# tusen-ai/SST

Hardware: AMD Instinct MI355X
Metric: LiDAR frames/sec (SST backbone fwd+bwd) at Waymo 0.32m voxels (higher is better)
Workload: dtype f32 (storage, accumulation, attention, LayerNorm, reductions: fp32; the dense products of the encoder layers from the EXACT three-way bf16 split of both fp32 operands, six bf16 MFMA products with fp32 accumulation - error vs float64 <= 2 x the fp32 matrix pipe's: tests/test_gpu_dense_f32x6.py)

## Files before the change

sst_amd/csrc/layer_exec.hip:

```cpp
#include <stdint.h>
#include "common.h"

namespace {

enum { kEpiBias = 0, kEpiGelu = 1, kEpiRelu = 2, kEpiMulGeluGrad = 3, kEpiMulReluGrad = 4, kEpiAdd = 5 };
constexpr int kC = 128, kFF = 256;

int64_t wg_ws(int64_t m, int which) {
  sst_wgrad_problem_f32 p[5];
  float* const any = (float*)(uintptr_t)256;
  for (auto& q : p) {
    q.dy = q.x = any;
    q.dw = q.db = any;
    q.m = m;
    q.x_add_rows = nullptr, q.x_add_index = nullptr;
  }
  if (which == 0 || which == 2) {
    p[0].ld_dy = kC, p[0].ld_x = kFF, p[0].out = kC, p[0].in = kFF;
    p[1].ld_dy = kFF, p[1].ld_x = kC, p[1].out = kFF, p[1].in = kC;
    if (which == 0) return sst_weight_grad_group_f32x6_workspace_bytes(p, 2);
    p[2].ld_dy = kC, p[2].ld_x = kC, p[2].out = kC, p[2].in = kC;
    p[3].ld_dy = 3 * kC, p[3].ld_x = kC, p[3].out = 2 * kC, p[3].in = kC;
    p[4].ld_dy = 3 * kC, p[4].ld_x = kC, p[4].out = kC, p[4].in = kC;
    return sst_weight_grad_group_f32x6_workspace_bytes(p, 5);
// ... 1 lines not shown
  p[0].ld_dy = kC, p[0].ld_x = kC, p[0].out = kC, p[0].in = kC;
  p[1].ld_dy = 3 * kC, p[1].ld_x = kC, p[1].out = 2 * kC, p[1].in = kC;
  p[2].ld_dy = 3 * kC, p[2].ld_x = kC, p[2].out = kC, p[2].in = kC;
  return sst_weight_grad_group_f32x6_workspace_bytes(p, 3);
}

int64_t wg_ws_bf16(int64_t m) {
  sst_wgrad_problem_bf16 p[5];
  for (auto& q : p) q.m = m;
  p[0].p = 2 * kC, p[1].p = kC, p[2].p = kC, p[3].p = kFF, p[4].p = kFF;
  return sst_wgrad_group_workspace_bytes(p, 5);
}

}

extern "C" {

int64_t sst_encoder_layer_bwd_workspace_bytes(int64_t m, int n_heads) {
  if (m < 0 || n_heads < 1) return SST_ERR_ARG;
  const int64_t a = sst_encoder_tail_bwd_workspace_bytes(m), d = sst_sra_attn_bwd_workspace_bytes(m, n_heads), e = wg_ws(m, 2);
  if (a < 0 || d < 0 || e < 0) return SST_ERR_UNSUPPORTED;
  return sst_align_up(a, 256) + sst_align_up(e, 256) + sst_align_up(d, 256) + 256;
}

int64_t sst_encoder_layer_wpack_bytes(void) { return sst_encoder_tail_pack_bytes(); }

int sst_encoder_layer_fwd_f32x6(const sst_encoder_layer_fwd_args* a, void* stream) {
  if (!a || a->m < 0 || a->n_heads * 16 != kC || (a->act != 1 && a->act != 2)) return SST_ERR_ARG;
  if (a->m == 0) return SST_OK;
  if (!a->x || !a->qkv || !a->o || !a->lse || !a->y1 || !a->st1 || !a->pre || !a->h || !a->s2 || !a->y2 || !a->st2)
    return SST_ERR_ARG;
  if (!a->xp && (!a->xpos_table || !a->xpos_idx)) return SST_ERR_ARG;
  const int64_t m = a->m;
  int rc;
  if (a->xp == nullptr)
    rc = sst_inproj_pos_f32x6(a->x, kC, a->xpos_table, a->xpos_idx, a->w_in, kC, a->b_in, m, a->qkv, 3 * kC, stream);
  else
    rc = sst_tall_linear_epi2_f32x6(a->xp, a->x, 2 * kC, kC, a->w_in, kC, 0, a->b_in, m, kC, 3 * kC, kEpiBias, nullptr, nullptr, 0,
                                    a->qkv, 3 * kC, stream);
  if (rc) return rc;
  if (a->head_scale != nullptr)
    rc = sst_sra_attn_cos_fwd_f32(a->qkv, a->qkv + kC, a->qkv + 2 * kC, 3 * kC, 3 * kC, 3 * kC, a->tok, a->winoff, a->order,
                                  a->n_windows, a->n_heads, a->head_scale, a->max_tokens, a->o, kC, a->lse, stream);
  else
    rc = sst_sra_attn_fwd_ord_f32(a->qkv, a->qkv + kC, a->qkv + 2 * kC, 3 * kC, 3 * kC, 3 * kC, a->tok, a->winoff, a->order,
                                  a->n_windows, a->n_heads, a->scale, a->max_tokens, a->impl, a->o, kC, a->lse, stream);
  if (rc) return rc;
  if (!a->wpack) return SST_ERR_ARG;
  if (a->w_out || a->w1 || a->w2) {
    rc = sst_encoder_tail_pack_f32x6(a->w_out, a->w1, a->w2, a->wpack, stream);
    if (rc) return rc;
  }
  sst_encoder_tail_fwd_args t;
  t.m = m, t.act = a->act, t.reserved = 0, t.eps = a->eps, t.reserved_f = 0.f;
  t.o = a->o, t.x = a->x, t.packed = a->wpack;
  t.b_out = a->b_out, t.b1 = a->b1, t.b2 = a->b2, t.n1w = a->n1w, t.n1b = a->n1b, t.n2w = a->n2w, t.n2b = a->n2b;
  t.pos_table = a->pos_table, t.pos_idx = a->pos_idx;
  t.s1 = a->s1, t.st1 = a->st1, t.y1 = a->y1, t.pre = a->pre, t.h = a->h, t.s2 = a->s2, t.st2 = a->st2, t.y2 = a->y2;
  t.y2p = a->pos_table != nullptr ? a->y2p : nullptr;
  return sst_encoder_tail_fwd_f32x6(&t, stream);
}

int sst_encoder_layer_bwd_f32x6(const sst_encoder_layer_bwd_args* a, void* stream) {
  if (!a || a->m < 0 || a->n_heads * 16 != kC || (a->act != 1 && a->act != 2)) return SST_ERR_ARG;
  if (a->m == 0) return SST_OK;
  if (!a->dy2 || !a->workspace || !a->ds2 || !a->dpre || !a->ds1 || !a->d_o || !a->dqkv || !a->wpack) return SST_ERR_ARG;
  if (!a->dn2w || !a->dn2b || !a->dn1w || !a->dn1b) return SST_ERR_ARG;
  if (!a->xp && (!a->xpos_table || !a->xpos_idx)) return SST_ERR_ARG;
  const int64_t m = a->m;
  char* ws = (char*)a->workspace;
  void* ws_tail = ws;
  ws += sst_align_up(sst_encoder_tail_bwd_workspace_bytes(m), 256);
  void* ws_wg = ws;
  ws += sst_align_up(wg_ws(m, 2), 256);
  void* ws_sra = ws;
  int rc;
  sst_encoder_tail_bwd_args t;
  t.m = m, t.act = a->act, t.reserved = 0;
  t.dy2 = a->dy2, t.dy2p = a->dy2p, t.s2 = a->s2, t.st2 = a->st2, t.pre = a->pre, t.s1 = a->s1, t.st1 = a->st1;
  t.packed = a->wpack, t.n1w = a->n1w, t.n2w = a->n2w;
  t.ds2 = a->ds2, t.dpre = a->dpre, t.ds1 = a->ds1, t.d_o = a->d_o;
  t.dn2w = a->dn2w, t.dn2b = a->dn2b, t.dn1w = a->dn1w, t.dn1b = a->dn1b;
  t.workspace = ws_tail;
  float *part2 = nullptr, *part1 = nullptr;
  int rows = 0;
  rc = sst_internal_encoder_tail_bwd_f32x6(&t, &part2, &part1, &rows, stream);
  if (rc) return rc;
  sst_colsum_rider riders[2];
  riders[0].partials = part2, riders[0].nb = rows, riders[0].width = 2 * kC, riders[0].split = kC;
  riders[0].out0 = a->dn2w, riders[0].out1 = a->dn2b;
  riders[1].partials = part1, riders[1].nb = rows, riders[1].width = 2 * kC, riders[1].split = kC;
  riders[1].out0 = a->dn1w, riders[1].out1 = a->dn1b;
  if (a->head_scale != nullptr)
    rc = sst_sra_attn_cos_bwd_f32(a->qkv, a->qkv + kC, a->qkv + 2 * kC, a->o, a->d_o, a->lse, 3 * kC, 3 * kC, 3 * kC, kC, kC, a->tok,
                                  a->winoff, a->order, a->n_windows, m, a->n_heads, a->head_scale, a->max_tokens, a->dqkv,
                                  a->dqkv + kC, a->dqkv + 2 * kC, 3 * kC, 3 * kC, 3 * kC, a->cos_r, stream);
  else
    rc = sst_sra_attn_bwd_ord_f32(a->qkv, a->qkv + kC, a->qkv + 2 * kC, a->o, a->d_o, a->lse, 3 * kC, 3 * kC, 3 * kC, kC, kC, a->tok,
                                  a->winoff, a->order, a->n_windows, m, a->n_heads, a->scale, a->max_tokens, a->impl, a->dqkv,
                                  a->dqkv + kC, a->dqkv + 2 * kC, 3 * kC, 3 * kC, 3 * kC, ws_sra, stream);
  if (rc) return rc;
  sst_wgrad_problem_f32 g[5];
  for (auto& q : g) q.x_add_rows = nullptr, q.x_add_index = nullptr;
  g[0].dy = a->ds2, g[0].x = a->h, g[0].m = m, g[0].ld_dy = kC, g[0].ld_x = kFF, g[0].dw = a->dw2, g[0].db = a->db2;
  g[0].out = kC, g[0].in = kFF;
  g[1].dy = a->dpre, g[1].x = a->y1, g[1].m = m, g[1].ld_dy = kFF, g[1].ld_x = kC, g[1].dw = a->dw1, g[1].db = a->db1;
  g[1].out = kFF, g[1].in = kC;
  g[2].dy = a->ds1, g[2].x = a->o, g[2].m = m, g[2].ld_dy = kC, g[2].ld_x = kC, g[2].dw = a->dwo, g[2].db = a->dbo;
  g[2].out = kC, g[2].in = kC;
  g[3].dy = a->dqkv, g[3].x = a->xp ? a->xp : a->x, g[3].m = m, g[3].ld_dy = 3 * kC, g[3].ld_x = kC, g[3].dw = a->dw_in;
  g[3].db = a->db_in, g[3].out = 2 * kC, g[3].in = kC;
  if (!a->xp) g[3].x_add_rows = a->xpos_table, g[3].x_add_index = a->xpos_idx;
  g[4].dy = a->dqkv + 2 * kC, g[4].x = a->x, g[4].m = m, g[4].ld_dy = 3 * kC, g[4].ld_x = kC;
  g[4].dw = a->dw_in + 2 * kC * kC, g[4].db = a->db_in + 2 * kC, g[4].out = kC, g[4].in = kC;
  rc = sst_internal_weight_grad_group_f32x6(g, 5, ws_wg, riders, 2, stream);
  if (rc) return rc;
  return sst_tall_linear_epi_f32x6(a->dqkv, 3 * kC, a->w_in, kC, 1, nullptr, m, 3 * kC, kC, kEpiAdd, a->ds1, nullptr, kC, a->ds1, kC,
                                   stream);
}

int64_t sst_encoder_layer_bwd_bf16_workspace_bytes(int64_t m) {
  if (m < 0) return SST_ERR_ARG;
  const int64_t a = sst_encoder_tail_bwd_bf16_workspace_bytes(m), b = wg_ws_bf16(m);
  if (a < 0 || b < 0) return SST_ERR_UNSUPPORTED;
  return sst_align_up(a, 256) + sst_align_up(b, 256) + 256;
}

int sst_encoder_layer_fwd_bf16(const sst_encoder_layer_fwd_bf16_args* a, void* stream) {
  if (!a || a->m < 0 || a->n_heads * 16 != kC || (a->act != 1 && a->act != 2)) return SST_ERR_ARG;
  if (a->m == 0) return SST_OK;
  if (!a->x || !a->xp || !a->wqk || !a->wv || !a->wout || !a->w1 || !a->w2 || !a->qk || !a->v || !a->o || !a->lse || !a->y1 ||
// ... 92 lines not shown
```

sst_amd/csrc/layer_tail_x6.hip:

```cpp
#include <math.h>
#include <stdlib.h>
#include "common.h"

#ifndef SST_NT_OUT
#define SST_NT_OUT false
#endif
#ifndef SST_NT_BWD
#define SST_NT_BWD true
#endif

namespace {

typedef float f32x4 __attribute__((ext_vector_type(4)));
typedef float f32x2 __attribute__((ext_vector_type(2)));
typedef unsigned u32x4 __attribute__((ext_vector_type(4)));
typedef __bf16 bf16x8 __attribute__((ext_vector_type(8)));
typedef __bf16 bf16x2 __attribute__((ext_vector_type(2)));

__device__ __forceinline__ unsigned pack2(float lo, float hi) {
  const f32x2 v = {lo, hi};
  return __builtin_bit_cast(unsigned, __builtin_convertvector(v, bf16x2));
}
__device__ __forceinline__ float lo_f(unsigned p) { return __uint_as_float(p << 16); }
__device__ __forceinline__ float hi_f(unsigned p) { return __uint_as_float(p & 0xffff0000u); }
__device__ __forceinline__ f32x4 mma32(u32x4 a, u32x4 b, f32x4 c) {
  return __builtin_amdgcn_mfma_f32_16x16x32_bf16(__builtin_bit_cast(bf16x8, a), __builtin_bit_cast(bf16x8, b), c, 0, 0, 0);
}
__device__ __forceinline__ void split2(float a, float b, unsigned& p0, unsigned& p1, unsigned& p2) {
  p0 = pack2(a, b);
  const float ra = a - lo_f(p0), rb = b - hi_f(p0);
  p1 = pack2(ra, rb);
  p2 = pack2(ra - lo_f(p1), rb - hi_f(p1));
}
struct img3 {
  u32x4 p0, p1, p2;
};
__device__ __forceinline__ img3 split8(const f32x4& a, const f32x4& b) {
  unsigned q0[4], q1[4], q2[4];
  split2(a[0], a[1], q0[0], q1[0], q2[0]);
  split2(a[2], a[3], q0[1], q1[1], q2[1]);
  split2(b[0], b[1], q0[2], q1[2], q2[2]);
  split2(b[2], b[3], q0[3], q1[3], q2[3]);
  img3 r;
  r.p0 = (u32x4){q0[0], q0[1], q0[2], q0[3]};
  r.p1 = (u32x4){q1[0], q1[1], q1[2], q1[3]};
  r.p2 = (u32x4){q2[0], q2[1], q2[2], q2[3]};
  return r;
}
__device__ __forceinline__ void join8(const img3& v, f32x4& a, f32x4& b) {
#pragma unroll
  for (int i = 0; i < 2; ++i) {
    a[2 * i] = (lo_f(v.p2[i]) + lo_f(v.p1[i])) + lo_f(v.p0[i]);
    a[2 * i + 1] = (hi_f(v.p2[i]) + hi_f(v.p1[i])) + hi_f(v.p0[i]);
    b[2 * i] = (lo_f(v.p2[2 + i]) + lo_f(v.p1[2 + i])) + lo_f(v.p0[2 + i]);
    b[2 * i + 1] = (hi_f(v.p2[2 + i]) + hi_f(v.p1[2 + i])) + hi_f(v.p0[2 + i]);
  }
}

__device__ __forceinline__ float erf_as(float z, float& e) {
  const float az = fabsf(z);
  const float t = __builtin_amdgcn_rcpf(fmaf(0.3275911f, az, 1.f));
  e = __expf(-az * az);
  const float poly = t * fmaf(t, fmaf(t, fmaf(t, fmaf(t, 1.061405429f, -1.453152027f), 1.421413741f), -0.284496736f), 0.254829592f);
  return copysignf(fmaf(-poly, e, 1.f), z);
}
__device__ __forceinline__ float gelu_f(float x) {
  float e;
  return 0.5f * x * (1.f + erf_as(x * 0.70710678118654752f, e));
}
__device__ __forceinline__ float gelu_grad_f(float x) {
  float e;
  const float phi = 0.5f * (1.f + erf_as(x * 0.70710678118654752f, e));
  return fmaf(x * 0.3989422804014327f, e, phi);
}

__device__ __forceinline__ int w_lds_row(int n) {
  const int tp = n >> 5, within = n & 31;
  return 16 * (2 * tp + ((within >> 2) & 1)) + ((within >> 3) << 2) + (within & 3);
}

template <int CTRL>
__device__ __forceinline__ float dpp_add(float v) {
  return v + __int_as_float(__builtin_amdgcn_update_dpp(0, __float_as_int(v), CTRL, 0xf, 0xf, false));
}
__device__ __forceinline__ float row_sum16(float v) {
  v = dpp_add<0xB1>(v);
  v = dpp_add<0x4E>(v);
  v = dpp_add<0x141>(v);
  return dpp_add<0x140>(v);
}

constexpr int kC = 128, kFF = 256, kHC = 32, kNF = kFF / kHC;
constexpr int kFrag = 1024;
constexpr int kI1 = 2 * 4 * kFrag;
constexpr int kI2 = 8 * 1 * kFrag;
constexpr int kIA = 8 * 2 * kFrag;
constexpr int kPart1 = 3 * kI1, kPart2 = 3 * kI2;
constexpr int kSlot = kPart1 + kPart2;
static_assert(3 * kIA <= kSlot, "slot");
#ifndef SST_TAIL_WAVES
#define SST_TAIL_WAVES 4
#endif
constexpr int kWaves = SST_TAIL_WAVES, kNTH = 64 * kWaves, kRowsPerWg = 16 * kWaves;
static_assert(kNTH >= 2 * kC, "one thread per LayerNorm parameter-gradient column");
constexpr int kNChunks = kNF + 2;
constexpr int kPackDir = kNChunks * kSlot;
constexpr int kParF = 6 * kC + kFF;
constexpr int kArea = kSlot;
constexpr int kScr = 2048;
constexpr int kLdsFwd = kArea + kParF * 4 + kWaves * kScr;
constexpr int kLdsBwd = kArea + 2 * kC * 4 + kWaves * 2 * kC * 4 + kWaves * kScr;

struct tail_weights {
  const float* wo;
  const float* w1;
  const float* w2;
};

template <bool BWD>
__device__ __forceinline__ void stage_load(const tail_weights W, int chunk, int t, float (&r)[16]) {
  if (!BWD) {
    if (chunk < 2) {
#pragma unroll
      for (int u = 0; u < 2; ++u) {
        const int idx = t + 512 * u, n = idx >> 3, k8 = (idx & 7) * 8;
        const float* p = W.wo + n * kC + 64 * chunk + k8;
// ... 54 lines not shown
  *(u32x4*)(base + 2 * image_bytes + off) = s.p2;
}

template <bool BWD>
__device__ __forceinline__ void stage_store(unsigned char* slot, int chunk, int t, const float (&r)[16]) {
  const bool outproj = BWD ? chunk >= kNF : chunk < 2;
  if (outproj) {
#pragma unroll
    for (int u = 0; u < 2; ++u) {
      const int idx = t + 512 * u;
      const int n = BWD ? (idx & 127) : (idx >> 3), k8 = BWD ? (idx >> 7) * 8 : (idx & 7) * 8;
      store_images(slot, kIA, frag_off(w_lds_row(n), k8, 2), r + 8 * u);
    }
  } else {
    const int n1 = BWD ? (t & 31) : (t >> 4), k1 = BWD ? (t >> 5) * 8 : (t & 15) * 8;
    store_images(slot, kI1, frag_off(w_lds_row(n1), k1, 4), r);
    const int n2 = BWD ? (t & 127) : (t >> 2), k2 = BWD ? (t >> 7) * 8 : (t & 3) * 8;
    store_images(slot + kPart1, kI2, frag_off(w_lds_row(n2), k2, 1), r + 8);
  }
}

constexpr int kPackMany = 16;
struct pack_batch {
  tail_weights w[kPackMany];
  unsigned char* dst[kPackMany];
};
__global__ __launch_bounds__(512) void encoder_tail_pack_k(const pack_batch B) {
  extern __shared__ __attribute__((aligned(16))) unsigned char lds[];
  const int layer = blockIdx.x / (2 * kNChunks), blk = blockIdx.x % (2 * kNChunks);
  const tail_weights W = B.w[layer];
  const int chunk = blk % kNChunks, dir = blk / kNChunks;
  float r[16];
  if (dir == 0) {
    stage_load<false>(W, chunk, threadIdx.x, r);
    stage_store<false>(lds, chunk, threadIdx.x, r);
  } else {
    stage_load<true>(W, chunk, threadIdx.x, r);
    stage_store<true>(lds, chunk, threadIdx.x, r);
  }
  __syncthreads();
  unsigned char* dst = B.dst[layer] + (size_t)blk * kSlot;
  for (int i = threadIdx.x; i < kSlot / 16; i += 512) *(u32x4*)(dst + 16 * i) = *(const u32x4*)(lds + 16 * i);
}

__device__ __forceinline__ void dma_pieces(const unsigned char* __restrict__ src, unsigned char* dst, int pieces, int wave, int lane) {
  for (int i = wave; i < pieces; i += kWaves)
    __builtin_amdgcn_global_load_lds((const __attribute__((address_space(1))) void*)(src + i * 1024 + lane * 16),
                                     (__attribute__((address_space(3))) void*)(dst + i * 1024), 16, 0, 0);
}

__device__ __forceinline__ void barrier_lds_only() { asm volatile("s_waitcnt lgkmcnt(0)\n\ts_barrier" ::: "memory"); }
__device__ __forceinline__ void barrier_drain() { asm volatile("s_waitcnt vmcnt(0) lgkmcnt(0)\n\ts_barrier" ::: "memory"); }

struct tile_io {
  unsigned char* scr;
  int frag_off0;
  int row_off[2];
  int64_t rrow[2];
  bool rvalid[2];
  int rcol;
};
__device__ __forceinline__ tile_io make_tile_io(unsigned char* scr, int lane, int64_t r0, int64_t m) {
  tile_io t;
  const int c = lane & 15, g = lane >> 4;
  t.scr = scr;
  t.frag_off0 = c * 128 + (((2 * g) ^ (c & 7)) << 4);
#pragma unroll
  for (int i = 0; i < 2; ++i) {
    const int r = 8 * i + (lane >> 3), p = lane & 7;
    t.row_off[i] = r * 128 + ((p ^ (r & 7)) << 4);
    t.rvalid[i] = r0 + r < m;
    t.rrow[i] = t.rvalid[i] ? r0 + r : m - 1;
  }
  t.rcol = (lane & 7) * 4;
  return t;
}
template <bool STREAM>
__device__ __forceinline__ void store32(const tile_io& t, float* __restrict__ base, int64_t ld, int col0, const f32x4& v0,
                                        const f32x4& v1) {
  *(f32x4*)(t.scr + t.frag_off0) = v0;
  *(f32x4*)(t.scr + (t.frag_off0 ^ 16)) = v1;
#pragma unroll
  for (int i = 0; i < 2; ++i) {
    const f32x4 w = *(const f32x4*)(t.scr + t.row_off[i]);
    if (t.rvalid[i]) {
      if (STREAM)
        __builtin_nontemporal_store(w, (f32x4*)(base + t.rrow[i] * ld + col0 + t.rcol));
      else
        *(f32x4*)(base + t.rrow[i] * ld + col0 + t.rcol) = w;
    }
  }
}
__device__ __forceinline__ void load32_issue(const tile_io& t, const float* __restrict__ base, int64_t ld, int col0, f32x4 (&w)[2]) {
#pragma unroll
  for (int i = 0; i < 2; ++i) w[i] = *(const f32x4*)(base + t.rrow[i] * ld + col0 + t.rcol);
}
__device__ __forceinline__ void load32_finish(const tile_io& t, const f32x4 (&w)[2], f32x4& v0, f32x4& v1) {
#pragma unroll
  for (int i = 0; i < 2; ++i) *(f32x4*)(t.scr + t.row_off[i]) = w[i];
  v0 = *(const f32x4*)(t.scr + t.frag_off0);
  v1 = *(const f32x4*)(t.scr + (t.frag_off0 ^ 16));
}

template <int HALF>
__device__ __forceinline__ void mma_half(const unsigned char* slot, int lane_off, const f32x4 (&x)[4][2], f32x4 (&acc)[8]) {
#pragma unroll
  for (int s2 = 0; s2 < 2; ++s2) {
    const img3 xs = split8(x[2 * HALF + s2][0], x[2 * HALF + s2][1]);
#pragma unroll
    for (int t0 = 0; t0 < 8; t0 += 4) {
      u32x4 a0[4], a1[4], a2[4];
#pragma unroll
      for (int u = 0; u < 4; ++u) {
        const int off = lane_off + ((t0 + u) * 2 + s2) * kFrag;
        a0[u] = *(const u32x4*)(slot + off);
        a1[u] = *(const u32x4*)(slot + kIA + off);
        a2[u] = *(const u32x4*)(slot + 2 * kIA + off);
      }
#pragma unroll
      for (int u = 0; u < 4; ++u) acc[t0 + u] = mma32(a0[u], xs.p2, acc[t0 + u]);
#pragma unroll
      for (int u = 0; u < 4; ++u) acc[t0 + u] = mma32(a2[u], xs.p0, acc[t0 + u]);
#pragma unroll
      for (int u = 0; u < 4; ++u) acc[t0 + u] = mma32(a1[u], xs.p1, acc[t0 + u]);
#pragma unroll
      for (int u = 0; u < 4; ++u) acc[t0 + u] = mma32(a0[u], xs.p1, acc[t0 + u]);
#pragma unroll
      for (int u = 0; u < 4; ++u) acc[t0 + u] = mma32(a1[u], xs.p0, acc[t0 + u]);
#pragma unroll
      for (int u = 0; u < 4; ++u) acc[t0 + u] = mma32(a0[u], xs.p0, acc[t0 + u]);
    }
  }
}

__device__ __forceinline__ f32x4 add4(const f32x4& a, const f32x4& b) {
  return (f32x4){a[0] + b[0], a[1] + b[1], a[2] + b[2], a[3] + b[3]};
}

__device__ __forceinline__ void mma_first(const unsigned char* slot, int lane_off1, const img3 (&y)[4], f32x4& out0, f32x4& out1) {
  const f32x4 z = {0.f, 0.f, 0.f, 0.f};
  f32x4 am[2] = {z, z}, ca[2] = {z, z}, cb[2] = {z, z};
#pragma unroll
  for (int s = 0; s < 4; ++s) {
    u32x4 a0[2], a1[2], a2[2];
#pragma unroll
    for (int T = 0; T < 2; ++T) {
      const int off = lane_off1 + (T * 4 + s) * kFrag;
      a0[T] = *(const u32x4*)(slot + off);
      a1[T] = *(const u32x4*)(slot + kI1 + off);
      a2[T] = *(const u32x4*)(slot + 2 * kI1 + off);
// ... 27 lines not shown
      a2[u] = *(const u32x4*)(slot2 + 2 * kI2 + off);
    }
#pragma unroll
    for (int u = 0; u < 4; ++u) acc[t0 + u] = mma32(a0[u], h.p2, acc[t0 + u]);
#pragma unroll
    for (int u = 0; u < 4; ++u) acc[t0 + u] = mma32(a2[u], h.p0, acc[t0 + u]);
#pragma unroll
    for (int u = 0; u < 4; ++u) acc[t0 + u] = mma32(a1[u], h.p1, acc[t0 + u]);
#pragma unroll
    for (int u = 0; u < 4; ++u) acc[t0 + u] = mma32(a0[u], h.p1, acc[t0 + u]);
#pragma unroll
    for (int u = 0; u < 4; ++u) acc[t0 + u] = mma32(a1[u], h.p0, acc[t0 + u]);
#pragma unroll
    for (int u = 0; u < 4; ++u) acc[t0 + u] = mma32(a0[u], h.p0, acc[t0 + u]);
  }
}

__device__ __forceinline__ void ln_stats(f32x4 (&v)[4][2], float eps, float& mean, float& rstd) {
  float sum = 0.f;
#pragma unroll
  for (int s = 0; s < 4; ++s)
#pragma unroll
    for (int r = 0; r < 4; ++r) sum += v[s][0][r] + v[s][1][r];
  sum += __shfl_xor(sum, 16, 64);
  sum += __shfl_xor(sum, 32, 64);
  mean = sum * (1.f / 128.f);
  float sq = 0.f;
#pragma unroll
  for (int s = 0; s < 4; ++s)
#pragma unroll
    for (int h = 0; h < 2; ++h)
#pragma unroll
      for (int r = 0; r < 4; ++r) {
        v[s][h][r] -= mean;
        sq = fmaf(v[s][h][r], v[s][h][r], sq);
      }
  sq += __shfl_xor(sq, 16, 64);
  sq += __shfl_xor(sq, 32, 64);
  rstd = rsqrtf(sq * (1.f / 128.f) + eps);
}

struct tail_fwd_params {
  const float *o, *x;
  const unsigned char* packed;
  const float *b_out, *b1, *b2, *n1w, *n1b, *n2w, *n2b;
  float eps;
  int64_t m;
  float *s1, *st1, *y1, *pre, *h, *s2, *st2, *y2;
  const float* pos_table;
  const int32_t* pos_idx;
  float* y2p;
};

template <int ACT>
__global__ __launch_bounds__(kNTH, 2) void encoder_tail_fwd_x6_k(const tail_fwd_params P) {
  extern __shared__ __attribute__((aligned(16))) unsigned char lds[];
  float* par = (float*)(lds + kArea);
  const int lane = threadIdx.x & 63, g = lane >> 4, c = lane & 15, wave = threadIdx.x >> 6;
  const int64_t r0 = (int64_t)blockIdx.x * kRowsPerWg + wave * 16;
  const bool valid = r0 + c < P.m;
  const int64_t row = valid ? r0 + c : P.m - 1;
  const tile_io io = make_tile_io(lds + kArea + kParF * 4 + wave * kScr, lane, r0, P.m);
  const unsigned char* packed = P.packed;
  unsigned char* const part2 = lds + kPart1;
  dma_pieces(packed, lds, 3 * kIA / 1024, wave, lane);
  f32x4 ob[4][2], xr[4][2];
  {
    f32x4 wo[4][2], wx[4][2];
#pragma unroll
    for (int s = 0; s < 4; ++s) load32_issue(io, P.o, kC, 32 * s, wo[s]);
#pragma unroll
    for (int s = 0; s < 4; ++s) load32_issue(io, P.x, kC, 32 * s, wx[s]);
#pragma unroll
    for (int s = 0; s < 4; ++s) load32_finish(io, wo[s], ob[s][0], ob[s][1]);
#pragma unroll
    for (int s = 0; s < 4; ++s) load32_finish(io, wx[s], xr[s][0], xr[s][1]);
  }
  for (int i = threadIdx.x; i < kC; i += kNTH) {
    par[i] = P.b_out ? P.b_out[i] : 0.f;
    par[kC + i] = P.n1w[i];
    par[2 * kC + i] = P.n1b[i];
    par[3 * kC + i] = P.b2 ? P.b2[i] : 0.f;
    par[4 * kC + i] = P.n2w[i];
    par[5 * kC + i] = P.n2b[i];
  }
  for (int i = threadIdx.x; i < kFF; i += kNTH) par[6 * kC + i] = P.b1 ? P.b1[i] : 0.f;

  const int lane_offA = lane * 16, lane_off1 = lane * 16, lane_off2 = lane * 16;
  const f32x4 z4 = {0.f, 0.f, 0.f, 0.f};
  f32x4 acc[8];
#pragma unroll
  for (int T = 0; T < 8; ++T) acc[T] = z4;
  img3 yi[4];

  barrier_drain();
  mma_half<0>(lds, lane_offA, ob, acc);
  barrier_drain();
  dma_pieces(packed + kSlot, lds, 3 * kIA / 1024, wave, lane);
  barrier_drain();
  mma_half<1>(lds, lane_offA, ob, acc);
  barrier_drain();
  dma_pieces(packed + 2 * kSlot, lds, kSlot / 1024, wave, lane);
  {
    f32x4 v[4][2];
#pragma unroll
    for (int s = 0; s < 4; ++s) {
      const int n0 = 32 * s + 8 * g;
      v[s][0] = acc[2 * s] + *(const f32x4*)(par + n0) + xr[s][0];
      v[s][1] = acc[2 * s + 1] + *(const f32x4*)(par + n0 + 4) + xr[s][1];
      if (P.s1 != nullptr) store32<true>(io, P.s1, kC, 32 * s, v[s][0], v[s][1]);
    }
    float mean, rstd;
    ln_stats(v, P.eps, mean, rstd);
    if (valid && g == 0) ((float2*)P.st1)[row] = make_float2(mean, rstd);
#pragma unroll
    for (int s = 0; s < 4; ++s) {
      const int n0 = 32 * s + 8 * g;
      const f32x4 y0 = v[s][0] * rstd * *(const f32x4*)(par + kC + n0) + *(const f32x4*)(par + 2 * kC + n0);
      const f32x4 y1 = v[s][1] * rstd * *(const f32x4*)(par + kC + n0 + 4) + *(const f32x4*)(par + 2 * kC + n0 + 4);
      store32<true>(io, P.y1, kC, 32 * s, y0, y1);
      yi[s] = split8(y0, y1);
    }
#pragma unroll
    for (int T = 0; T < 8; ++T) acc[T] = z4;
  }
  barrier_drain();
  f32x4 sp0 = z4, sp1 = z4, sh0 = z4, sh1 = z4;
#pragma unroll 1
  for (int j = 0; j < kNF; ++j) {
    if (j > 0) {
      store32<true>(io, P.pre, kFF, kHC * (j - 1), sp0, sp1);
      store32<true>(io, P.h, kFF, kHC * (j - 1), sh0, sh1);
    }
    f32x4 p0, p1;
    mma_first(lds, lane_off1, yi, p0, p1);
    const int nl = kHC * j + 8 * g;
    p0 = add4(p0, *(const f32x4*)(par + 6 * kC + nl));
    p1 = add4(p1, *(const f32x4*)(par + 6 * kC + nl + 4));
    f32x4 h0, h1;
#pragma unroll
    for (int r = 0; r < 4; ++r) {
      h0[r] = ACT == 1 ? gelu_f(p0[r]) : fmaxf(p0[r], 0.f);
      h1[r] = ACT == 1 ? gelu_f(p1[r]) : fmaxf(p1[r], 0.f);
    }
    const img3 hs = split8(h0, h1);
    barrier_drain();
    if (j + 1 < kNF) dma_pieces(packed + (size_t)(j + 3) * kSlot, lds, kPart1 / 1024, wave, lane);
    mma_second(part2, lane_off2, hs, acc);
    sp0 = p0, sp1 = p1, sh0 = h0, sh1 = h1;
    barrier_drain();
    if (j + 1 < kNF) dma_pieces(packed + (size_t)(j + 3) * kSlot + kPart1, part2, kPart2 / 1024, wave, lane);
  }
  store32<true>(io, P.pre, kFF, kHC * (kNF - 1), sp0, sp1);
  store32<true>(io, P.h, kFF, kHC * (kNF - 1), sh0, sh1);
  f32x4 v[4][2];
#pragma unroll
  for (int s = 0; s < 4; ++s) {
    const int n0 = 32 * s + 8 * g;
    f32x4 ya, yb;
    join8(yi[s], ya, yb);
    v[s][0] = acc[2 * s] + *(const f32x4*)(par + 3 * kC + n0) + ya;
    v[s][1] = acc[2 * s + 1] + *(const f32x4*)(par + 3 * kC + n0 + 4) + yb;
    if (P.s2 != nullptr) store32<true>(io, P.s2, kC, 32 * s, v[s][0], v[s][1]);
  }
  float mean, rstd;
  ln_stats(v, P.eps, mean, rstd);
  if (valid && g == 0) ((float2*)P.st2)[row] = make_float2(mean, rstd);
  const float* prow = P.pos_table != nullptr ? P.pos_table + (size_t)P.pos_idx[row] * kC : nullptr;
#pragma unroll
  for (int s = 0; s < 4; ++s) {
    const int n0 = 32 * s + 8 * g;
    const f32x4 y0 = v[s][0] * rstd * *(const f32x4*)(par + 4 * kC + n0) + *(const f32x4*)(par + 5 * kC + n0);
    const f32x4 y1 = v[s][1] * rstd * *(const f32x4*)(par + 4 * kC + n0 + 4) + *(const f32x4*)(par + 5 * kC + n0 + 4);
    store32<SST_NT_OUT>(io, P.y2, kC, 32 * s, y0, y1);
    if (prow != nullptr) store32<SST_NT_OUT>(io, P.y2p, kC, 32 * s, y0 + *(const f32x4*)(prow + n0), y1 + *(const f32x4*)(prow + n0 + 4));
  }
}

struct tail_bwd_params {
  const float *dy2, *dy2p, *s2, *st2, *n2w, *pre, *s1, *st1, *n1w;
  const unsigned char* packed;
  int64_t m;
  float *ds2, *dpre, *ds1, *d_o;
  float *part2, *part1;
};

__device__ __forceinline__ void ln_bwd(f32x4 (&d)[4][2], f32x4 (&sv)[4][2], const float2 st, const float* gamma, int g, int c,
                                       bool valid, float* red) {
  float sg = 0.f, sgx = 0.f;
#pragma unroll
  for (int s = 0; s < 4; ++s)
#pragma unroll
    for (int h = 0; h < 2; ++h) {
      const f32x4 w = *(const f32x4*)(gamma + 32 * s + 8 * g + 4 * h);
      sv[s][h] = (sv[s][h] - st.x) * st.y;
      f32x4 a, b;
#pragma unroll
      for (int r = 0; r < 4; ++r) {
        a[r] = row_sum16(valid ? d[s][h][r] * sv[s][h][r] : 0.f);
        b[r] = row_sum16(valid ? d[s][h][r] : 0.f);
      }
      if (c == 0) {
        *(f32x4*)(red + 32 * s + 8 * g + 4 * h) = a;
        *(f32x4*)(red + kC + 32 * s + 8 * g + 4 * h) = b;
      }
      d[s][h] *= w;
#pragma unroll
      for (int r = 0; r < 4; ++r) {
        sg += d[s][h][r];
        sgx = fmaf(d[s][h][r], sv[s][h][r], sgx);
      }
    }
  sg += __shfl_xor(sg, 16, 64);
  sg += __shfl_xor(sg, 32, 64);
  sgx += __shfl_xor(sgx, 16, 64);
  sgx += __shfl_xor(sgx, 32, 64);
  const float mg = sg * (1.f / 128.f), mgx = sgx * (1.f / 128.f);
#pragma unroll
  for (int s = 0; s < 4; ++s)
#pragma unroll
    for (int h = 0; h < 2; ++h)
#pragma unroll
      for (int r = 0; r < 4; ++r) d[s][h][r] = st.y * (d[s][h][r] - mg - sv[s][h][r] * mgx);
}

template <int ACT>
__global__ __launch_bounds__(kNTH, 2) void encoder_tail_bwd_x6_k(const tail_bwd_params P) {
  extern __shared__ __attribute__((aligned(16))) unsigned char lds[];
  float* par = (float*)(lds + kArea);
  float* red = par + 2 * kC;
  const int lane = threadIdx.x & 63, g = lane >> 4, c = lane & 15, wave = threadIdx.x >> 6;
  const int64_t r0 = (int64_t)blockIdx.x * kRowsPerWg + wave * 16;
  const bool valid = r0 + c < P.m;
  const int64_t row = valid ? r0 + c : P.m - 1;
  const tile_io io = make_tile_io(lds + kArea + 2 * kC * 4 + kWaves * 2 * kC * 4 + wave * kScr, lane, r0, P.m);
  const unsigned char* packed = P.packed;
  unsigned char* const part2 = lds + kPart1;
  dma_pieces(packed, lds, kSlot / 1024, wave, lane);
  f32x4 d[4][2], sv[4][2];
  {
    f32x4 wd[4][2], we[4][2];
#pragma unroll
    for (int s = 0; s < 4; ++s) load32_issue(io, P.dy2, kC, 32 * s, wd[s]);
    if (P.dy2p != nullptr) {
#pragma unroll
      for (int s = 0; s < 4; ++s) load32_issue(io, P.dy2p, kC, 32 * s, we[s]);
#pragma unroll
      for (int s = 0; s < 4; ++s) {
        wd[s][0] += we[s][0];
        wd[s][1] += we[s][1];
      }
    }
#pragma unroll
    for (int s = 0; s < 4; ++s) load32_issue(io, P.s2, kC, 32 * s, we[s]);
#pragma unroll
    for (int s = 0; s < 4; ++s) load32_finish(io, wd[s], d[s][0], d[s][1]);
#pragma unroll
    for (int s = 0; s < 4; ++s) load32_finish(io, we[s], sv[s][0], sv[s][1]);
  }
  const float2 st2 = ((const float2*)P.st2)[row];
  for (int i = threadIdx.x; i < kC; i += kNTH) {
    par[i] = P.n2w[i];
    par[kC + i] = P.n1w[i];
  }
  barrier_drain();

  img3 di[4];
  {
    ln_bwd(d, sv, st2, par, g, c, valid, red + wave * 2 * kC);
#pragma unroll
    for (int s = 0; s < 4; ++s) {
      store32<SST_NT_BWD>(io, P.ds2, kC, 32 * s, d[s][0], d[s][1]);
      di[s] = split8(d[s][0], d[s][1]);
    }
  }
  const int lane_offA = lane * 16, lane_off1 = lane * 16, lane_off2 = lane * 16;
  const f32x4 z4 = {0.f, 0.f, 0.f, 0.f};
  f32x4 acc[8];
#pragma unroll
  for (int T = 0; T < 8; ++T) acc[T] = z4;
  f32x4 xs1[4][2];
  f32x4 pq[2];
  load32_issue(io, P.pre, kFF, 0, pq);

  f32x4 sd0 = z4, sd1 = z4;
  auto ffn_chunk = [&](int j, const f32x4 q0, const f32x4 q1) __attribute__((always_inline)) {
    if (j > 0) store32<SST_NT_BWD>(io, P.dpre, kFF, kHC * (j - 1), sd0, sd1);
    f32x4 p0, p1;
    mma_first(lds, lane_off1, di, p0, p1);
#pragma unroll
    for (int r = 0; r < 4; ++r) {
      p0[r] *= ACT == 1 ? gelu_grad_f(q0[r]) : (q0[r] > 0.f ? 1.f : 0.f);
      p1[r] *= ACT == 1 ? gelu_grad_f(q1[r]) : (q1[r] > 0.f ? 1.f : 0.f);
    }
    const img3 hs = split8(p0, p1);
    barrier_drain();
    if (j + 1 < kNF) dma_pieces(packed + (size_t)(j + 1) * kSlot, lds, kPart1 / 1024, wave, lane);
    mma_second(part2, lane_off2, hs, acc);
    sd0 = p0, sd1 = p1;
    barrier_drain();
    if (j + 1 < kNF)
      dma_pieces(packed + (size_t)(j + 1) * kSlot + kPart1, part2, kPart2 / 1024, wave, lane);
    else
      dma_pieces(packed + (size_t)kNF * kSlot, lds, 3 * kIA / 1024, wave, lane);
  };
  barrier_drain();
  if (threadIdx.x < 2 * kC) {
    float a = 0.f;
#pragma unroll
    for (int w = 0; w < kWaves; ++w) a += red[w * 2 * kC + threadIdx.x];
    P.part2[(int64_t)blockIdx.x * 2 * kC + threadIdx.x] = a;
  }
#pragma unroll 1
  for (int j = 0; j < kNF - 1; ++j) {
    f32x4 q0, q1;
    load32_finish(io, pq, q0, q1);
    load32_issue(io, P.pre, kFF, kHC * (j + 1), pq);
    ffn_chunk(j, q0, q1);
  }
  {
    f32x4 q0, q1;
    load32_finish(io, pq, q0, q1);
    ffn_chunk(kNF - 1, q0, q1);
    store32<SST_NT_BWD>(io, P.dpre, kFF, kHC * (kNF - 1), sd0, sd1);
    {
      f32x4 ws[4][2];
#pragma unroll
      for (int s = 0; s < 4; ++s) load32_issue(io, P.s1, kC, 32 * s, ws[s]);
#pragma unroll
      for (int s = 0; s < 4; ++s) load32_finish(io, ws[s], xs1[s][0], xs1[s][1]);
    }
    f32x4 dd[4][2];
#pragma unroll
    for (int s = 0; s < 4; ++s) {
      f32x4 ya, yb;
      join8(di[s], ya, yb);
      dd[s][0] = acc[2 * s] + ya;
      dd[s][1] = acc[2 * s + 1] + yb;
    }
    const float2 st1 = ((const float2*)P.st1)[row];
    barrier_drain();
    ln_bwd(dd, xs1, st1, par + kC, g, c, valid, red + wave * 2 * kC);
#pragma unroll
    for (int s = 0; s < 4; ++s) {
      store32<SST_NT_BWD>(io, P.ds1, kC, 32 * s, dd[s][0], dd[s][1]);
      xs1[s][0] = dd[s][0];
      xs1[s][1] = dd[s][1];
    }
#pragma unroll
    for (int T = 0; T < 8; ++T) acc[T] = z4;
    barrier_drain();
    mma_half<0>(lds, lane_offA, xs1, acc);
    barrier_drain();
    dma_pieces(packed + (size_t)(kNF + 1) * kSlot, lds, 3 * kIA / 1024, wave, lane);
    barrier_drain();
    mma_half<1>(lds, lane_offA, xs1, acc);
  }
#pragma unroll
  for (int s = 0; s < 4; ++s) store32<SST_NT_OUT>(io, P.d_o, kC, 32 * s, acc[2 * s], acc[2 * s + 1]);
  barrier_drain();
  if (threadIdx.x < 2 * kC) {
    float b = 0.f;
#pragma unroll
    for (int w = 0; w < kWaves; ++w) b += red[w * 2 * kC + threadIdx.x];
    P.part1[(int64_t)blockIdx.x * 2 * kC + threadIdx.x] = b;
  }
}

bool aligned16(const void* p) { return ((uintptr_t)p & 15) == 0; }

template <typename K>
int configure(K kernel, int lds_bytes, unsigned long long* mask) {
  if (sst_first_use_on_device(mask)) {
    SST_HIP(hipFuncSetAttribute((const void*)kernel, hipFuncAttributeMaxDynamicSharedMemorySize, lds_bytes));
    sst_mark_device(mask);
  }
  return SST_OK;
}

}

int sst_internal_encoder_tail_bwd_f32x6(const sst_encoder_tail_bwd_args* a, float** part2, float** part1, int* partial_rows,
                                        void* stream) {
  if (!a || a->m <= 0 || (a->act != 1 && a->act != 2)) return SST_ERR_ARG;
  const void* need[] = {a->dy2, a->s2, a->st2, a->n2w, a->pre, a->s1, a->st1, a->n1w, a->packed,
                        a->ds2, a->dpre, a->ds1, a->d_o, a->workspace};
  for (const void* p : need)
    if (!p || !aligned16(p)) return SST_ERR_ARG;
  if (a->dy2p && !aligned16(a->dy2p)) return SST_ERR_ARG;
  const int64_t rows = sst_div_up(a->m, (int64_t)kRowsPerWg);
  if (rows > 0x7fffffff / 2) return SST_ERR_UNSUPPORTED;
  tail_bwd_params P;
  P.dy2 = a->dy2, P.dy2p = a->dy2p, P.s2 = a->s2, P.st2 = a->st2, P.n2w = a->n2w, P.pre = a->pre, P.s1 = a->s1, P.st1 = a->st1;
  P.n1w = a->n1w, P.packed = (const unsigned char*)a->packed + kPackDir, P.m = a->m;
  P.ds2 = a->ds2, P.dpre = a->dpre, P.ds1 = a->ds1, P.d_o = a->d_o;
  P.part2 = (float*)a->workspace;
  P.part1 = P.part2 + rows * 2 * kC;
  hipStream_t st = (hipStream_t)stream;
  static unsigned long long cfg1 = 0, cfg2 = 0;
  if (a->act == 1) {
    const int rc = configure(encoder_tail_bwd_x6_k<1>, kLdsBwd, &cfg1);
    if (rc) return rc;
    hipLaunchKernelGGL(encoder_tail_bwd_x6_k<1>, dim3((unsigned)rows), dim3(kNTH), kLdsBwd, st, P);
  } else {
    const int rc = configure(encoder_tail_bwd_x6_k<2>, kLdsBwd, &cfg2);
    if (rc) return rc;
    hipLaunchKernelGGL(encoder_tail_bwd_x6_k<2>, dim3((unsigned)rows), dim3(kNTH), kLdsBwd, st, P);
  }
  SST_LAUNCH_CHECK();
  *part2 = P.part2, *part1 = P.part1, *partial_rows = (int)rows;
  return SST_OK;
}

namespace {
__global__ __launch_bounds__(1024) void tail_colsum_k(const float* __restrict__ partials, int nb, int width, float* __restrict__ out0,
                                                      float* __restrict__ out1, int split) {
  __shared__ float red[32][33];
  const int cx = threadIdx.x & 31, gy = threadIdx.x >> 5;
  const int i = blockIdx.x * 32 + cx;
  float acc = 0.f;
  if (i < width)
    for (int b = gy; b < nb; b += 32) acc += partials[(int64_t)b * width + i];
  red[gy][cx] = acc;
  __syncthreads();
  if (gy == 0 && i < width) {
    float t = 0.f;
#pragma unroll
    for (int k = 0; k < 32; ++k) t += red[k][cx];
    if (i < split)
      out0[i] = t;
    else
      out1[i - split] = t;
  }
}
}

extern "C" {

int64_t sst_encoder_tail_pack_bytes(void) { return 2 * (int64_t)kPackDir; }

int sst_encoder_tail_pack_f32x6_many(const float* const* d_w_out, const float* const* d_w1, const float* const* d_w2,
                                     void* const* d_packed, int n, void* stream) {
  if (n < 0 || (n > 0 && (!d_w_out || !d_w1 || !d_w2 || !d_packed))) return SST_ERR_ARG;
  static unsigned long long cfg = 0;
  const int rc = configure(encoder_tail_pack_k, kSlot, &cfg);
  if (rc) return rc;
  for (int base = 0; base < n; base += kPackMany) {
    pack_batch B;
    const int cnt = n - base < kPackMany ? n - base : kPackMany;
    for (int i = 0; i < cnt; ++i) {
      const float *wo = d_w_out[base + i], *w1 = d_w1[base + i], *w2 = d_w2[base + i];
      void* dst = d_packed[base + i];
      if (!wo || !w1 || !w2 || !dst || !aligned16(wo) || !aligned16(w1) || !aligned16(w2) || !aligned16(dst)) return SST_ERR_ARG;
      B.w[i].wo = wo, B.w[i].w1 = w1, B.w[i].w2 = w2;
      B.dst[i] = (unsigned char*)dst;
    }
    hipLaunchKernelGGL(encoder_tail_pack_k, dim3(cnt * 2 * kNChunks), dim3(512), kSlot, (hipStream_t)stream, B);
  }
  SST_LAUNCH_CHECK();
  return SST_OK;
}

int sst_encoder_tail_pack_f32x6(const float* d_w_out, const float* d_w1, const float* d_w2, void* d_packed, void* stream) {
  return sst_encoder_tail_pack_f32x6_many(&d_w_out, &d_w1, &d_w2, &d_packed, 1, stream);
}

int64_t sst_encoder_tail_bwd_workspace_bytes(int64_t m) {
  if (m < 0) return SST_ERR_ARG;
  return sst_align_up(2 * sst_div_up(m > 0 ? m : 1, (int64_t)kRowsPerWg) * 2 * kC * (int64_t)sizeof(float), 256);
}

int sst_encoder_tail_fwd_f32x6(const sst_encoder_tail_fwd_args* a, void* stream) {
  if (!a || a->m < 0 || (a->act != 1 && a->act != 2)) return SST_ERR_ARG;
  if (a->m == 0) return SST_OK;
  const void* need[] = {a->o, a->x, a->packed, a->n1w, a->n1b, a->n2w, a->n2b, a->st1, a->y1, a->pre, a->h, a->st2, a->y2};
  for (const void* p : need)
    if (!p || !aligned16(p)) return SST_ERR_ARG;
  if ((a->s1 && !aligned16(a->s1)) || (a->s2 && !aligned16(a->s2))) return SST_ERR_ARG;
  if ((a->pos_table != nullptr) != (a->pos_idx != nullptr) || (a->pos_table != nullptr) != (a->y2p != nullptr)) return SST_ERR_ARG;
  if (a->pos_table && (!aligned16(a->pos_table) || !aligned16(a->y2p))) return SST_ERR_ARG;
  tail_fwd_params P;
  P.o = a->o, P.x = a->x, P.packed = (const unsigned char*)a->packed;
  P.b_out = a->b_out, P.b1 = a->b1, P.b2 = a->b2, P.n1w = a->n1w, P.n1b = a->n1b, P.n2w = a->n2w, P.n2b = a->n2b;
  P.eps = a->eps, P.m = a->m;
  P.s1 = a->s1, P.st1 = a->st1, P.y1 = a->y1, P.pre = a->pre, P.h = a->h, P.s2 = a->s2, P.st2 = a->st2, P.y2 = a->y2;
  P.pos_table = a->pos_table, P.pos_idx = a->pos_idx, P.y2p = a->y2p;
  const int64_t rows = sst_div_up(a->m, (int64_t)kRowsPerWg);
  if (rows > 0x7fffffff) return SST_ERR_UNSUPPORTED;
  hipStream_t st = (hipStream_t)stream;
  static unsigned long long cfg1 = 0, cfg2 = 0;
  if (a->act == 1) {
    const int rc = configure(encoder_tail_fwd_x6_k<1>, kLdsFwd, &cfg1);
    if (rc) return rc;
    hipLaunchKernelGGL(encoder_tail_fwd_x6_k<1>, dim3((unsigned)rows), dim3(kNTH), kLdsFwd, st, P);
  } else {
    const int rc = configure(encoder_tail_fwd_x6_k<2>, kLdsFwd, &cfg2);
    if (rc) return rc;
    hipLaunchKernelGGL(encoder_tail_fwd_x6_k<2>, dim3((unsigned)rows), dim3(kNTH), kLdsFwd, st, P);
  }
  SST_LAUNCH_CHECK();
  return SST_OK;
}

int sst_encoder_tail_bwd_f32x6(const sst_encoder_tail_bwd_args* a, void* stream) {
  if (!a || a->m < 0) return SST_ERR_ARG;
  if (!a->dn2w || !a->dn2b || !a->dn1w || !a->dn1b) return SST_ERR_ARG;
  hipStream_t st = (hipStream_t)stream;
  if (a->m == 0) {
    for (float* p : {a->dn2w, a->dn2b, a->dn1w, a->dn1b}) SST_HIP(hipMemsetAsync(p, 0, sizeof(float) * kC, st));
    return SST_OK;
  }
  float *part2 = nullptr, *part1 = nullptr;
  int rows = 0;
  const int rc = sst_internal_encoder_tail_bwd_f32x6(a, &part2, &part1, &rows, stream);
  if (rc) return rc;
  hipLaunchKernelGGL(tail_colsum_k, dim3(2 * kC / 32), dim3(1024), 0, st, part2, rows, 2 * kC, a->dn2w, a->dn2b, kC);
  hipLaunchKernelGGL(tail_colsum_k, dim3(2 * kC / 32), dim3(1024), 0, st, part1, rows, 2 * kC, a->dn1w, a->dn1b, kC);
  SST_LAUNCH_CHECK();
  return SST_OK;
}

}
```

Before: 102.0.

## Cache activation derivative in forward pass and use 32-bit row offsets in tail I/O

When training (s1 present), the forward tail kernel computes the GELU/ReLU derivative along with the activation and overwrites the pre-activation buffer with it. The backward kernel then multiplies by the stored derivative instead of recomputing erf/exp. Separately, tile I/O gets a narrow mode that uses precomputed 32-bit byte offsets instead of 64-bit row*ld address math, falling back to the wide mode for large m. The pre buffer now holds a derivative instead of the pre-activation, which couples the forward and backward passes through the reserved flag and doubles the number of kernel instantiations.

```diff
diff --git a/sst_amd/csrc/layer_exec.hip b/sst_amd/csrc/layer_exec.hip
--- a/sst_amd/csrc/layer_exec.hip
+++ b/sst_amd/csrc/layer_exec.hip
@@ -77,7 +77,7 @@
     if (rc) return rc;
   }
   sst_encoder_tail_fwd_args t;
-  t.m = m, t.act = a->act, t.reserved = 0, t.eps = a->eps, t.reserved_f = 0.f;
+  t.m = m, t.act = a->act, t.reserved = a->s1 != nullptr ? 1 : 0, t.eps = a->eps, t.reserved_f = 0.f;
   t.o = a->o, t.x = a->x, t.packed = a->wpack;
   t.b_out = a->b_out, t.b1 = a->b1, t.b2 = a->b2, t.n1w = a->n1w, t.n1b = a->n1b, t.n2w = a->n2w, t.n2b = a->n2b;
   t.pos_table = a->pos_table, t.pos_idx = a->pos_idx;
@@ -101,7 +101,7 @@
   void* ws_sra = ws;
   int rc;
   sst_encoder_tail_bwd_args t;
-  t.m = m, t.act = a->act, t.reserved = 0;
+  t.m = m, t.act = a->act, t.reserved = 1;
   t.dy2 = a->dy2, t.dy2p = a->dy2p, t.s2 = a->s2, t.st2 = a->st2, t.pre = a->pre, t.s1 = a->s1, t.st1 = a->st1;
   t.packed = a->wpack, t.n1w = a->n1w, t.n2w = a->n2w;
   t.ds2 = a->ds2, t.dpre = a->dpre, t.ds1 = a->ds1, t.d_o = a->d_o;
diff --git a/sst_amd/csrc/layer_tail_x6.hip b/sst_amd/csrc/layer_tail_x6.hip
--- a/sst_amd/csrc/layer_tail_x6.hip
+++ b/sst_amd/csrc/layer_tail_x6.hip
@@ -72,6 +72,13 @@
   float e;
   const float phi = 0.5f * (1.f + erf_as(x * 0.70710678118654752f, e));
   return fmaf(x * 0.3989422804014327f, e, phi);
+}
+
+__device__ __forceinline__ void gelu_both_f(float x, float& h, float& g) {
+  float e;
+  const float er = erf_as(x * 0.70710678118654752f, e);
+  h = 0.5f * x * (1.f + er);
+  g = fmaf(x * 0.3989422804014327f, e, 0.5f * (1.f + er));
 }
 
 __device__ __forceinline__ int w_lds_row(int n) {
@@ -232,16 +239,27 @@
 __device__ __forceinline__ void barrier_lds_only() { asm volatile("s_waitcnt lgkmcnt(0)\n\ts_barrier" ::: "memory"); }
 __device__ __forceinline__ void barrier_drain() { asm volatile("s_waitcnt vmcnt(0) lgkmcnt(0)\n\ts_barrier" ::: "memory"); }
 
+typedef __attribute__((address_space(1))) char* gchars;
+typedef __attribute__((address_space(1))) f32x4 gf32x4;
+template <bool WIDE>
 struct tile_io {
   unsigned char* scr;
   int frag_off0;
   int row_off[2];
   int64_t rrow[2];
+  mutable unsigned roff[2][2];
   bool rvalid[2];
   int rcol;
+  __device__ __forceinline__ gf32x4* at(const float* base, int64_t ld, int col0, int i) const {
+    if (WIDE) return (gf32x4*)(base + rrow[i] * ld + col0 + rcol);
+    unsigned& off = roff[ld == kFF ? 1 : 0][i];
+    asm volatile("" : "+v"(off));
+    return (gf32x4*)((gchars)base + 4 * col0 + off);
+  }
 };
-__device__ __forceinline__ tile_io make_tile_io(unsigned char* scr, int lane, int64_t r0, int64_t m) {
-  tile_io t;
+template <bool WIDE>
+__device__ __forceinline__ tile_io<WIDE> make_tile_io(unsigned char* scr, int lane, int64_t r0, int64_t m) {
+  tile_io<WIDE> t;
   const int c = lane & 15, g = lane >> 4;
   t.scr = scr;
   t.frag_off0 = c * 128 + (((2 * g) ^ (c & 7)) << 4);
@@ -251,12 +269,14 @@
     t.row_off[i] = r * 128 + ((p ^ (r & 7)) << 4);
     t.rvalid[i] = r0 + r < m;
     t.rrow[i] = t.rvalid[i] ? r0 + r : m - 1;
+    t.roff[0][i] = ((unsigned)t.rrow[i] * (unsigned)kC + 4u * (lane & 7)) * 4u;
+    t.roff[1][i] = ((unsigned)t.rrow[i] * (unsigned)kFF + 4u * (lane & 7)) * 4u;
   }
   t.rcol = (lane & 7) * 4;
   return t;
 }
-template <bool STREAM>
-__device__ __forceinline__ void store32(const tile_io& t, float* __restrict__ base, int64_t ld, int col0, const f32x4& v0,
+template <bool STREAM, bool WIDE>
+__device__ __forceinline__ void store32(const tile_io<WIDE>& t, float* __restrict__ base, int64_t ld, int col0, const f32x4& v0,
                                         const f32x4& v1) {
   *(f32x4*)(t.scr + t.frag_off0) = v0;
   *(f32x4*)(t.scr + (t.frag_off0 ^ 16)) = v1;
@@ -265,17 +285,19 @@
     const f32x4 w = *(const f32x4*)(t.scr + t.row_off[i]);
     if (t.rvalid[i]) {
       if (STREAM)
-        __builtin_nontemporal_store(w, (f32x4*)(base + t.rrow[i] * ld + col0 + t.rcol));
+        __builtin_nontemporal_store(w, t.at(base, ld, col0, i));
       else
-        *(f32x4*)(base + t.rrow[i] * ld + col0 + t.rcol) = w;
-    }
-  }
-}
-__device__ __forceinline__ void load32_issue(const tile_io& t, const float* __restrict__ base, int64_t ld, int col0, f32x4 (&w)[2]) {
-#pragma unroll
-  for (int i = 0; i < 2; ++i) w[i] = *(const f32x4*)(base + t.rrow[i] * ld + col0 + t.rcol);
-}
-__device__ __forceinline__ void load32_finish(const tile_io& t, const f32x4 (&w)[2], f32x4& v0, f32x4& v1) {
+        *t.at(base, ld, col0, i) = w;
+    }
+  }
+}
+template <bool WIDE>
+__device__ __forceinline__ void load32_issue(const tile_io<WIDE>& t, const float* __restrict__ base, int64_t ld, int col0, f32x4 (&w)[2]) {
+#pragma unroll
+  for (int i = 0; i < 2; ++i) w[i] = *t.at(base, ld, col0, i);
+}
+template <bool WIDE>
+__device__ __forceinline__ void load32_finish(const tile_io<WIDE>& t, const f32x4 (&w)[2], f32x4& v0, f32x4& v1) {
 #pragma unroll
   for (int i = 0; i < 2; ++i) *(f32x4*)(t.scr + t.row_off[i]) = w[i];
   v0 = *(const f32x4*)(t.scr + t.frag_off0);
@@ -409,15 +431,18 @@
   float* y2p;
 };
 
-template <int ACT>
+constexpr int kModeDact = 4, kModeWide = 8;
+template <int MODE>
 __global__ __launch_bounds__(kNTH, 2) void encoder_tail_fwd_x6_k(const tail_fwd_params P) {
+  constexpr int ACT = MODE & 3;
+  constexpr bool DACT = (MODE & kModeDact) != 0, WIDE = (MODE & kModeWide) != 0;
   extern __shared__ __attribute__((aligned(16))) unsigned char lds[];
   float* par = (float*)(lds + kArea);
   const int lane = threadIdx.x & 63, g = lane >> 4, c = lane & 15, wave = threadIdx.x >> 6;
   const int64_t r0 = (int64_t)blockIdx.x * kRowsPerWg + wave * 16;
   const bool valid = r0 + c < P.m;
   const int64_t row = valid ? r0 + c : P.m - 1;
-  const tile_io io = make_tile_io(lds + kArea + kParF * 4 + wave * kScr, lane, r0, P.m);
+  const tile_io<WIDE> io = make_tile_io<WIDE>(lds + kArea + kParF * 4 + wave * kScr, lane, r0, P.m);
   const unsigned char* packed = P.packed;
   unsigned char* const part2 = lds + kPart1;
   dma_pieces(packed, lds, 3 * kIA / 1024, wave, lane);
@@ -495,10 +520,26 @@
     p0 = add4(p0, *(const f32x4*)(par + 6 * kC + nl));
     p1 = add4(p1, *(const f32x4*)(par + 6 * kC + nl + 4));
     f32x4 h0, h1;
-#pragma unroll
-    for (int r = 0; r < 4; ++r) {
-      h0[r] = ACT == 1 ? gelu_f(p0[r]) : fmaxf(p0[r], 0.f);
-      h1[r] = ACT == 1 ? gelu_f(p1[r]) : fmaxf(p1[r], 0.f);
+    if (DACT) {
+#pragma unroll
+      for (int r = 0; r < 4; ++r) {
+        const float a0 = p0[r], a1 = p1[r];
+        if (ACT == 1) {
+          float ha, ga, hb, gb;
+          gelu_both_f(a0, ha, ga);
+          gelu_both_f(a1, hb, gb);
+          h0[r] = ha, p0[r] = ga, h1[r] = hb, p1[r] = gb;
+        } else {
+          h0[r] = fmaxf(a0, 0.f), p0[r] = a0 > 0.f ? 1.f : 0.f;
+          h1[r] = fmaxf(a1, 0.f), p1[r] = a1 > 0.f ? 1.f : 0.f;
+        }
+      }
+    } else {
+#pragma unroll
+      for (int r = 0; r < 4; ++r) {
+        h0[r] = ACT == 1 ? gelu_f(p0[r]) : fmaxf(p0[r], 0.f);
+        h1[r] = ACT == 1 ? gelu_f(p1[r]) : fmaxf(p1[r], 0.f);
+      }
     }
     const img3 hs = split8(h0, h1);
     barrier_drain();
@@ -581,8 +622,10 @@
       for (int r = 0; r < 4; ++r) d[s][h][r] = st.y * (d[s][h][r] - mg - sv[s][h][r] * mgx);
 }
 
-template <int ACT>
+template <int MODE>
 __global__ __launch_bounds__(kNTH, 2) void encoder_tail_bwd_x6_k(const tail_bwd_params P) {
+  constexpr int ACT = MODE & 3;
+  constexpr bool DACT = (MODE & kModeDact) != 0, WIDE = (MODE & kModeWide) != 0;
   extern __shared__ __attribute__((aligned(16))) unsigned char lds[];
   float* par = (float*)(lds + kArea);
   float* red = par + 2 * kC;
@@ -590,7 +633,7 @@
   const int64_t r0 = (int64_t)blockIdx.x * kRowsPerWg + wave * 16;
   const bool valid = r0 + c < P.m;
   const int64_t row = valid ? r0 + c : P.m - 1;
-  const tile_io io = make_tile_io(lds + kArea + 2 * kC * 4 + kWaves * 2 * kC * 4 + wave * kScr, lane, r0, P.m);
+  const tile_io<WIDE> io = make_tile_io<WIDE>(lds + kArea + 2 * kC * 4 + kWaves * 2 * kC * 4 + wave * kScr, lane, r0, P.m);
   const unsigned char* packed = P.packed;
   unsigned char* const part2 = lds + kPart1;
   dma_pieces(packed, lds, kSlot / 1024, wave, lane);
@@ -647,8 +690,8 @@
     mma_first(lds, lane_off1, di, p0, p1);
 #pragma unroll
     for (int r = 0; r < 4; ++r) {
-      p0[r] *= ACT == 1 ? gelu_grad_f(q0[r]) : (q0[r] > 0.f ? 1.f : 0.f);
-      p1[r] *= ACT == 1 ? gelu_grad_f(q1[r]) : (q1[r] > 0.f ? 1.f : 0.f);
+      p0[r] *= DACT ? q0[r] : ACT == 1 ? gelu_grad_f(q0[r]) : (q0[r] > 0.f ? 1.f : 0.f);
+      p1[r] *= DACT ? q1[r] : ACT == 1 ? gelu_grad_f(q1[r]) : (q1[r] > 0.f ? 1.f : 0.f);
     }
     const img3 hs = split8(p0, p1);
     barrier_drain();
@@ -735,11 +778,41 @@
   return SST_OK;
 }
 
+int tail_mode(int act, int reserved, int64_t m) {
+  return act | ((reserved & 1) ? kModeDact : 0) | (m * 384 * 4 < ((int64_t)1 << 31) ? 0 : kModeWide);
+}
+
+template <bool FWD, int MODE, typename PARAMS>
+int launch_one(const PARAMS& P, unsigned rows, hipStream_t st) {
+  static unsigned long long cfg = 0;
+  if constexpr (FWD) {
+    const int rc = configure(encoder_tail_fwd_x6_k<MODE>, kLdsFwd, &cfg);
+    if (rc) return rc;
+    hipLaunchKernelGGL(encoder_tail_fwd_x6_k<MODE>, dim3(rows), dim3(kNTH), kLdsFwd, st, P);
+  } else {
+    const int rc = configure(encoder_tail_bwd_x6_k<MODE>, kLdsBwd, &cfg);
+    if (rc) return rc;
+    hipLaunchKernelGGL(encoder_tail_bwd_x6_k<MODE>, dim3(rows), dim3(kNTH), kLdsBwd, st, P);
+  }
+  return SST_OK;
+}
+template <bool FWD, typename PARAMS>
+int launch_mode(int mode, const PARAMS& P, unsigned rows, hipStream_t st) {
+  switch (mode) {
+#define SST_TAIL_MODE(M) \
+  case M: return launch_one<FWD, M>(P, rows, st);
+    SST_TAIL_MODE(1) SST_TAIL_MODE(2) SST_TAIL_MODE(5) SST_TAIL_MODE(6)
+    SST_TAIL_MODE(9) SST_TAIL_MODE(10) SST_TAIL_MODE(13) SST_TAIL_MODE(14)
+#undef SST_TAIL_MODE
+  }
+  return SST_ERR_ARG;
+}
+
 }
 
 int sst_internal_encoder_tail_bwd_f32x6(const sst_encoder_tail_bwd_args* a, float** part2, float** part1, int* partial_rows,
                                         void* stream) {
-  if (!a || a->m <= 0 || (a->act != 1 && a->act != 2)) return SST_ERR_ARG;
+  if (!a || a->m <= 0 || (a->act != 1 && a->act != 2) || (a->reserved & ~1)) return SST_ERR_ARG;
   const void* need[] = {a->dy2, a->s2, a->st2, a->n2w, a->pre, a->s1, a->st1, a->n1w, a->packed,
                         a->ds2, a->dpre, a->ds1, a->d_o, a->workspace};
   for (const void* p : need)
@@ -753,17 +826,8 @@
   P.ds2 = a->ds2, P.dpre = a->dpre, P.ds1 = a->ds1, P.d_o = a->d_o;
   P.part2 = (float*)a->workspace;
   P.part1 = P.part2 + rows * 2 * kC;
-  hipStream_t st = (hipStream_t)stream;
-  static unsigned long long cfg1 = 0, cfg2 = 0;
-  if (a->act == 1) {
-    const int rc = configure(encoder_tail_bwd_x6_k<1>, kLdsBwd, &cfg1);
-    if (rc) return rc;
-    hipLaunchKernelGGL(encoder_tail_bwd_x6_k<1>, dim3((unsigned)rows), dim3(kNTH), kLdsBwd, st, P);
-  } else {
-    const int rc = configure(encoder_tail_bwd_x6_k<2>, kLdsBwd, &cfg2);
-    if (rc) return rc;
-    hipLaunchKernelGGL(encoder_tail_bwd_x6_k<2>, dim3((unsigned)rows), dim3(kNTH), kLdsBwd, st, P);
-  }
+  const int rc = launch_mode<false>(tail_mode(a->act, a->reserved, a->m), P, (unsigned)rows, (hipStream_t)stream);
+  if (rc) return rc;
   SST_LAUNCH_CHECK();
   *part2 = P.part2, *part1 = P.part1, *partial_rows = (int)rows;
   return SST_OK;
@@ -828,7 +892,7 @@
 }
 
 int sst_encoder_tail_fwd_f32x6(const sst_encoder_tail_fwd_args* a, void* stream) {
-  if (!a || a->m < 0 || (a->act != 1 && a->act != 2)) return SST_ERR_ARG;
+  if (!a || a->m < 0 || (a->act != 1 && a->act != 2) || (a->reserved & ~1)) return SST_ERR_ARG;
   if (a->m == 0) return SST_OK;
   const void* need[] = {a->o, a->x, a->packed, a->n1w, a->n1b, a->n2w, a->n2b, a->st1, a->y1, a->pre, a->h, a->st2, a->y2};
   for (const void* p : need)
@@ -844,17 +908,8 @@
   P.pos_table = a->pos_table, P.pos_idx = a->pos_idx, P.y2p = a->y2p;
   const int64_t rows = sst_div_up(a->m, (int64_t)kRowsPerWg);
   if (rows > 0x7fffffff) return SST_ERR_UNSUPPORTED;
-  hipStream_t st = (hipStream_t)stream;
-  static unsigned long long cfg1 = 0, cfg2 = 0;
-  if (a->act == 1) {
-    const int rc = configure(encoder_tail_fwd_x6_k<1>, kLdsFwd, &cfg1);
-    if (rc) return rc;
-    hipLaunchKernelGGL(encoder_tail_fwd_x6_k<1>, dim3((unsigned)rows), dim3(kNTH), kLdsFwd, st, P);
-  } else {
-    const int rc = configure(encoder_tail_fwd_x6_k<2>, kLdsFwd, &cfg2);
-    if (rc) return rc;
-    hipLaunchKernelGGL(encoder_tail_fwd_x6_k<2>, dim3((unsigned)rows), dim3(kNTH), kLdsFwd, st, P);
-  }
+  const int rc = launch_mode<true>(tail_mode(a->act, a->reserved, a->m), P, (unsigned)rows, (hipStream_t)stream);
+  if (rc) return rc;
   SST_LAUNCH_CHECK();
   return SST_OK;
 }
```

Result: no change. 102.5, median of 2 (+0.5%).
